# indrajeetadityaroy9/vit-inductive-bias-distillation

Hardware: AMD Instinct MI355X
Metric: distillation images/sec (BASD loss fwd+bwd+grad all-reduce), DeiT-S<-ResNet-50 @ bs256/GPU (higher is better)
Workload: dtype f32; 1 GPU; cfg2 DeiT-S<-ResNet-50 224x224; per_gpu_batch=256, global_batch=256, input_dtype=float32, layout=strided (CLS-sliced / channel-major views), backward=True, grad_allreduce_bytes=88202672, grad_allreduce=none at world size 1 (bucket packed, nothing to exchange), rank_readback=auto, readback_deferred_steps=1756, selector=basd_selector_chain mode 0, parallelism=dp1

## Files before the change

### include/basd_hip.h

```cpp
#ifndef BASD_HIP_H
#define BASD_HIP_H

#include <stdint.h>

#ifdef __cplusplus
extern "C" {
#endif

#ifndef __HIP_PLATFORM_AMD__
typedef struct ihipStream_t* hipStream_t;
#endif

#define BASD_OK 0
#define BASD_EINVAL (-1)
#define BASD_EUNSUPPORTED (-2)
#define BASD_DTYPE_F32 0
#define BASD_DTYPE_BF16 1
#define BASD_DTYPE_U8 2


int basd_gemm_nt(const void* a, int a_dtype, long a_sb, long a_sn, long a_sd, int a_rows_per_batch,
                 long a_batch_stride, const float* b, long ldb, long b_batch_stride, int M, int N, int K, int batch,
                 float* c, long ldc, long c_batch_stride, float scale, const float* bias, float beta,
                 float* colsum_part, float* col_mean, hipStream_t stream);
// ... 80 lines not shown

int basd_grassmann_distance_padded(const float* colnorm, int stride, int n_valid, const int* k_arr, const float* sw,
                                   int sw_stride, const int* sw_index, int items, float* d_out, hipStream_t stream);

int basd_sqrt_clamp(const float* in, float* out, long count, hipStream_t stream);

int basd_gram_finish(const float* c, const float* zbar, int n, int batch, long m_rows, float* out_u, float* out_c,
                     hipStream_t stream);

int basd_selector_tail(const float* t_d, const float* t_e, const float* t_tau, const float* t_vh, const float* t_vals,
                       const float* s_d, const float* s_e, const float* s_tau, const float* s_vh, const float* s_vals,
                       int d_s, int E, int L, int kmax, const int* ranks, const float* proj_s_t, float* z_s,
                       float* v_s, float* z_t, float* u_t, float* u_rot, float* sw, float* cos, int* k_arr,
                       const int* sw_index, float* sigma, int* flags, float* d_out, hipStream_t stream);

int basd_tridiag_mp_rank_rank1(const float* d, const float* e, const float* w, int n, int batch, double rho,
                               double factor, int cap, int* rank_out, const int* status, int* host_mirror,
                               hipStream_t stream);

int basd_tridiag_ranked_gated(float* a, long a_batch_stride, int n, int batch, float* d, float* e, float* tau, float* vh,
                              void* work, int rank_count, double factor, int cap, int* rank_out, int* host_mirror,
                              const unsigned* go_flag, unsigned go_value, int go_budget, hipStream_t stream);
int basd_flag_set(unsigned* flag, unsigned value, hipStream_t stream);

typedef struct BasdSelectorChain {
    const void* const* teacher_host_ptrs;
    long t_dtype, t_sb, t_sn, t_sd;
    const void* const* student_ptrs;
    long s_dtype, s_sb, s_sn, s_sd, s_vec_ok;
    const float* proj_t;
    const float* proj_s_t;
    long E, L, B, n_s, n_t, d_s, d_t;
    double mp_factor;
    long rank_cap;
    long kmax, kmax_cap, mode;
    float* z; float* z_sums; const void* const* z_ptrs; float* z_means; float* t_slabs; long t_splits;
    float* s_partial; float* s_means; float* s_slabs; long s_splits, s_parts;
    float* grams; float* d; float* e; float* tau; float* vh; float* vals; void* tri_work; void* tri_work_s;
    int* ranks; int* host_mirror;
    int* student_status_mirror;
    float* zv; float* vecs; float* u_rot; float* sw; float* cos; float* sigma; float* d_out;
    int* k_arr; const int* sw_index; int* jflags;
    hipStream_t main_stream, chain_stream, student_stream, tail_stream;
    void* ev_fork; void* ev_student; void* ev_ranks; void* ev_tail; void* ev_slot_free; void* ev_tgram; void* ev_tg0;
    hipStream_t fact_stream; unsigned* go_flag; long go_value; long go_budget;
    void* tm_proj; void* tm_tgram; void* tm_scol0; void* tm_scol1; void* tm_sgram; void* tm_tri0; void* tm_mid; void* tm_spec;
    hipStream_t cert_stream; int* cert_mirror; void* ev_cert;
    double* cert_scratch;
} BasdSelectorChain;
int basd_selector_chain(const BasdSelectorChain* args);
int basd_rank_certificate(const float* grams, const float* zbar, int n, int batch, double factor, double* scratch,
                          int* flag, hipStream_t stream);
long basd_rank_certificate_scratch_bytes(int batch);
int basd_debug_fill_lds(unsigned pattern, hipStream_t stream);
int basd_selector_chain_tail(const BasdSelectorChain* args, int kmax, int exact_k);
int basd_jacobi_lds_square_fits(int n);


int basd_token_weights(const void* const* attn_ptrs, int dtype, const float* mix, int L, long sb, long sh, long sq,
                       long sk, int B, int H, int A, int has_cls, int n_a, int n_t, int n_s, const int* atap0,
                       const int* atap1, const float* alam, const int* tap0, const int* tap1, const float* lam,
                       float* omega, float* omega_t, float* raw_out, hipStream_t stream);

int basd_student_project(const void* x, int dtype, long sb, long sn, int B, int n_s, int n_t, int D,
                         const float* omega, const int* tap0, const int* tap1, const float* lam, const int* range0,
                         const int* range1, float* mu, float* tr_s, float* a_prime, hipStream_t stream);

int basd_teacher_center(const void* const* tok_ptrs, int dtype, const float* mix, int L, long sb, long sn, long sd,
                        int B, int n, int D, const int* g0, const int* g1, const float* glam, const float* omega_t,
                        float* mu, float* tc, hipStream_t stream);
int basd_teacher_center_multi(const void* const* tok_ptrs, int dtype, const float* mix, int L, int G, long sb, long sn,
                              long sd, int B, int n, int D, const int* g0, const int* g1, const float* glam,
                              const float* omega_t, float* mu, float* tc, hipStream_t stream);
long basd_teacher_center_stream_scratch_floats(int G, int B, int n, int D);
int basd_teacher_center_stream(const void* const* tok_ptrs, int dtype, const float* mix, int L, int G, long sb, long sn,
                               long sd, int B, int n, int D, const int* g0, const int* g1, const float* glam,
                               const float* omega_t, float* mu, float* tc, float* scratch, hipStream_t stream);

int basd_gram_f64(const float* p, long p_batch_stride, int n, int D, int batch, double* g, long g_batch_stride,
                  hipStream_t stream);

int basd_gram_f64_split(const float* p, long p_batch_stride, int n, int D, int batch, int splits, double* slabs,
                        double* g, hipStream_t stream);

int basd_chol_f64(const double* g, long g_batch_stride, int n, int batch, double* l, long l_batch_stride,
                  hipStream_t stream);

int basd_stack_product(const double* la, const double* lb, long l_batch_stride, int n, int batch, int lb_period,
                       float* w, long w_batch_stride, hipStream_t stream);

int basd_procrustes_finalize(const float* w, long w_batch_stride, const float* sigma, int n, int n_s, int batch,
                             int t_period ,
                             const double* gb, long g_batch_stride, const float* omega, const int* tap0,
                             const int* tap1, const float* lam, const float* tr_s_part, int tr_slabs, float* tr_s,
                             float* tr_t, float* nuc, float* loss, float* k_prime, hipStream_t stream);

int basd_student_project_multi(const void* const* x_ptrs, int dtype, long sb, long sn, int E, int B, int n_s, int n_t,
                               int D, int ptrs_16B_aligned, const float* omega, long omega_e_stride, const int* tap0,
                               const int* tap1, const float* lam, const int* range0, const int* range1, float* mu,
                               float* tr_s, float* a_prime, hipStream_t stream);
int basd_student_grad_multi(const void* const* x_ptrs, int dtype, long sb, long sn, int E, int B, int n_s, int n_t,
                            int D, const float* omega, long omega_e_stride, const float* mu, const float* h,
                            const int* tap0, const int* tap1, const float* lam, const float* scale_ptr,
                            float scale_const, float* dx, const float* tnorm2, float* gomega, hipStream_t stream);
int basd_student_grad_fused(const void* const* x_ptrs, int dtype, long sb, long sn, int E, int B, int n_s, int n_t,
                            int D, int ptrs_16B_aligned, const float* omega, long omega_e_stride, const float* mu,
                            const float* k_prime, const float* a_prime, const int* tap0, const int* tap1,
                            const float* lam, const float* scale_ptr, float scale_const, float* dx,
                            hipStream_t stream);

typedef struct BasdProcrustesArgs {
    const void* const* student_ptrs;
    const void* const* student_host_ptrs;
    long s_dtype, s_sb, s_sn, s_aligned;
    const void* const* tok_ptrs;
    long t_dtype, t_sb, t_sn, t_sd;
    const void* const* attn_ptrs;
    long a_dtype, a_sb, a_sh, a_sq, a_sk;
    const float* mix;
    long E, L, G, B, n_s, n_t, d_s, d_t, H, A, has_cls, n_a, n, max_sweeps;
    const int* atap0; const int* atap1; const float* alam;
    const int* tap0; const int* tap1; const float* lam; const int* range0; const int* range1;
    const int* g0; const int* g1; const float* glam;
    float* omega; float* omega_t; float* raw; float* mu_t; float* tc; float* mu_s; float* tr_part; float* tr_s;
    float* a_prime;
    double* g_all; double* l_all;
    float* W; float* sigma; int* jflags; int* sweeps;
    float* tr_t; float* nuc; float* loss_b; float* k_prime;
    float* h; float* dx; const float* grad_layers;
    double* g_slabs; long g_splits;
    const float* uw_ce; float* uw_out;
    void* jac_ws;
    float* w_stack; float* sigma_u;
} BasdProcrustesArgs;
int basd_procrustes_forward_fused(const BasdProcrustesArgs* args, hipStream_t stream);
int basd_procrustes_tuning(int transposed_cores);

int basd_stack_product_t(const double* la, const double* lb, long l_batch_stride, int n, int batch, int lb_period,
                         float* w, long w_batch_stride, hipStream_t stream);
int basd_kprime_from_transposed(const float* w, long w_batch_stride, const float* sigma, int n, int batch,
                                const double* lb, long l_batch_stride, int lb_period, float* z, long z_batch_stride,
                                float* k_prime, hipStream_t stream);
int basd_procrustes_finish_transposed(const float* w, long w_batch_stride, const float* sigma, int n, int n_s,
                                      int batch, int t_period ,
                                      const double* gb, long g_batch_stride, const float* omega, const int* tap0,
                                      const int* tap1, const float* lam, const float* tr_s_part, int tr_slabs,
                                      float* tr_s, float* tr_t, float* nuc, float* loss, const double* lb,
                                      long l_batch_stride, int lb_period, float* k_prime, hipStream_t stream);
int basd_procrustes_finish_tuning(int fused);
int basd_ustack_stash(const float* wc, long wc_batch_stride, int n, int batch, float* w_stack, long w_stack_stride,
                      hipStream_t stream);
int basd_ustack_from_transposed(const float* x, long x_batch_stride, const float* sigma, int n, int batch,
                                float* w_stack, long w_stack_stride, float* scratch, long scratch_batch_stride,
                                float* sigma_u, int max_sweeps, int* jflags, hipStream_t stream);

int basd_scale_unless_one(float* x, long count, const float* num, const float* den, hipStream_t stream);

int basd_cross_entropy(const void* logits, int dtype, long ld, int B, int C, const long* labels, const float* probs,
                       long pld, float label_smoothing, long ignore_index, float* row_loss, float* dlogits,
                       hipStream_t stream);


int basd_event_create(void** out);
int basd_event_destroy(void* event);
int basd_stream_wait_event(hipStream_t stream, void* event);
int basd_event_record(void* event, hipStream_t stream);
// ... 134 lines not shown
```

### vit-inductive-bias-distillation_amd/basd_amd/_lib.py

```python
from __future__ import annotations

import ctypes as C
import os
import threading

_HERE = os.path.dirname(os.path.abspath(__file__))
LIB_PATH = os.path.join(_HERE, "libbasd_hip.so")

vp, i32, i64, f32, f64 = C.c_void_p, C.c_int, C.c_long, C.c_float, C.c_double

SIGNATURES = {
    "basd_gemm_nt": [vp, i32, i64, i64, i64, i32, i64, vp, i64, i64, i32, i32, i32, i32, vp, i64, i64, f32, vp, f32,
                     vp, vp, vp],
    "basd_gemm_tn_splits": [i32],
    "basd_gemm_tn": [vp, vp, i32, i64, i64, i64, i64, i64, i64, i64, i64, i32, i32, i32, i32, i32, vp, vp, i32, vp,
                     vp, i64, i64, f32, vp],
    "basd_colmean_parts": [i32],
    "basd_colmean": [vp, i32, i64, i64, i64, i32, i64, i32, i32, i32, i32, vp, vp, vp],
    "basd_colmean_multi": [vp, i32, i64, i64, i64, i32, i32, i32, i32, i32, vp, vp, i32, vp],
    "basd_syrk_splits": [i32, i32, i32],
    "basd_syrk_multi": [vp, i32, i64, i64, i64, i32, i32, i32, i32, vp, vp, i32, vp, vp, i64, i32, vp, i32, i32, vp],
    "basd_jacobi_workspace_ints": [i32, i32],
    "basd_jacobi_twopass_workspace_bytes": [i32, i32, i32],
    "basd_jacobi_stacked_twopass": [vp, i64, i32, i32, vp, i32, i32, f32, vp, vp, vp],
    "basd_jacobi_tuning": [i32],
    "basd_jacobi_ordering": [i32],
    "basd_gemm_tuning": [i32],
    "basd_gemm_tuning_get": [],
    "basd_jacobi_onesided": [vp, i64, i32, i32, i32, i32, vp, vp, i32, i32, f32, vp, vp, vp],
    "basd_sort_extract": [vp, i64, i32, i32, i32, i32, vp, i32, vp, vp, i32, vp],
    "basd_tridiag_workspace_bytes": [i32, i32],
    "basd_tridiag_tuning": [i32, i32, i32, i32, i32, i32],
    "basd_tridiag": [vp, i64, i32, i32, vp, vp, vp, vp, vp, vp],
    "basd_tridiag_ranked": [vp, i64, i32, i32, vp, vp, vp, vp, vp, i32, f64, i32, vp, vp, vp, vp],
    "basd_tridiag_ranked_gated": [vp, i64, i32, i32, vp, vp, vp, vp, vp, i32, f64, i32, vp, vp, vp, C.c_uint, i32, vp],
    "basd_flag_set": [vp, C.c_uint, vp],
    "basd_scale_unless_one": [vp, i64, vp, vp, vp],
    "basd_event_create": [vp],
    "basd_event_destroy": [vp],
    "basd_stream_wait_event": [vp, vp],
    "basd_tridiag_eigenvalues": [vp, vp, i32, i32, vp, vp],
    "basd_tridiag_apply_q": [vp, vp, i32, i32, i32, vp, vp, i32, i32, vp],
    "basd_tridiag_shifted_solve": [vp, vp, vp, i32, i32, i32, i32, vp, vp, vp],
    "basd_tridiag_mp_rank": [vp, vp, i32, i32, f64, i32, vp, vp, vp, vp, vp],
    "basd_tridiag_mp_rank_rank1": [vp, vp, vp, i32, i32, f64, f64, i32, vp, vp, vp, vp],
    "basd_tridiag_eigenvectors": [vp, vp, vp, vp, vp, i32, i32, i32, vp, vp, i32, vp],
    "basd_mp_rank": [vp, i32, i32, f64, i32, vp, vp, vp],
    "basd_grassmann_distance": [vp, i32, vp, vp, i32, vp, i32, vp, vp, vp],
    "basd_grassmann_distance_padded": [vp, i32, i32, vp, vp, i32, vp, i32, vp, vp],
    "basd_selector_tail": [vp] * 10 + [i32, i32, i32, i32] + [vp] * 14 + [vp],
    "basd_sqrt_clamp": [vp, vp, i64, vp],
    "basd_gram_finish": [vp, vp, i32, i32, i64, vp, vp, vp],
    "basd_cross_entropy": [vp, i32, i64, i32, i32, vp, vp, i64, f32, i64, vp, vp, vp],
    "basd_token_weights": [vp, i32, vp, i32, i64, i64, i64, i64, i32, i32, i32, i32, i32, i32, i32, vp, vp, vp, vp,
                           vp, vp, vp, vp, vp, vp],
    "basd_student_project": [vp, i32, i64, i64, i32, i32, i32, i32, vp, vp, vp, vp, vp, vp, vp, vp, vp, vp],
    "basd_teacher_center": [vp, i32, vp, i32, i64, i64, i64, i32, i32, i32, vp, vp, vp, vp, vp, vp, vp],
    "basd_teacher_center_multi": [vp, i32, vp, i32, i32, i64, i64, i64, i32, i32, i32, vp, vp, vp, vp, vp, vp, vp],
    "basd_teacher_center_stream_scratch_floats": [i32, i32, i32, i32],
    "basd_teacher_center_stream": [vp, i32, vp, i32, i32, i64, i64, i64, i32, i32, i32, vp, vp, vp, vp, vp, vp, vp, vp],
    "basd_gram_f64": [vp, i64, i32, i32, i32, vp, i64, vp],
    "basd_gram_f64_split": [vp, i64, i32, i32, i32, i32, vp, vp, vp],
    "basd_chol_f64": [vp, i64, i32, i32, vp, i64, vp],
    "basd_stack_product": [vp, vp, i64, i32, i32, i32, vp, i64, vp],
    "basd_procrustes_finalize": [vp, i64, vp, i32, i32, i32, i32, vp, i64, vp, vp, vp, vp, vp, i32, vp, vp, vp, vp,
                                 vp, vp],
    "basd_student_project_multi": [vp, i32, i64, i64, i32, i32, i32, i32, i32, i32, vp, i64, vp, vp, vp, vp, vp, vp,
                                   vp, vp, vp],
    "basd_student_grad_multi": [vp, i32, i64, i64, i32, i32, i32, i32, i32, vp, i64, vp, vp, vp, vp, vp, vp, f32, vp,
                                vp, vp, vp],
    "basd_student_grad_fused": [vp, i32, i64, i64, i32, i32, i32, i32, i32, i32, vp, i64, vp, vp, vp, vp, vp, vp, vp,
                                f32, vp, vp],
    "basd_procrustes_forward_fused": [vp, vp],
    "basd_procrustes_tuning": [i32],
    "basd_jacobi_plain4_fits": [i32],
    "basd_stack_product_t": [vp, vp, i64, i32, i32, i32, vp, i64, vp],
    "basd_kprime_from_transposed": [vp, i64, vp, i32, i32, vp, i64, i32, vp, i64, vp, vp],
    "basd_procrustes_finish_transposed": [vp, i64, vp, i32, i32, i32, i32, vp, i64, vp, vp, vp, vp, vp, i32, vp, vp, vp,
                                          vp, vp, i64, i32, vp, vp],
    "basd_procrustes_finish_tuning": [i32],
    "basd_ustack_stash": [vp, i64, i32, i32, vp, i64, vp],
    "basd_ustack_from_transposed": [vp, i64, vp, i32, i32, vp, i64, vp, i64, vp, i32, vp, vp],
    "basd_resample_tokens": [vp, i32, i64, i64, i64, i32, i32, i32, i32, vp, vp, vp, vp, vp],
    "basd_resample_tokens_adjoint": [vp, i32, i32, i32, i32, vp, vp, vp, vp, vp, vp, vp],
    "basd_teacher_factor": [vp, i64, vp, i32, i32, i32, vp, vp, i64, vp, vp, vp, vp, vp, vp, vp, vp, vp],
    "basd_teacher_factor_tiled": [vp, i64, vp, i32, i32, i32, vp, vp, i64, vp, vp, vp, vp, vp, vp, vp, vp, vp, vp],
    "basd_mix_grad_tokens": [vp, vp, i32, i32, i64, i64, i64, i32, i32, i32, i32, vp, vp, vp, vp, vp],
    "basd_mix_grad_tokens_scratch_floats": [i32, i32, i32, i32],
    "basd_mix_grad_tokens_onepass": [vp, vp, i32, i32, i64, i64, i64, i32, i32, i32, i32, vp, vp, vp, vp, vp, vp],
    "basd_token_weight_bwd": [vp, vp, i32, i32, i32, i32, vp, vp, vp, vp, vp, vp, i32, i32, i64, i64, i64, i64, i32,
                              i32, i32, vp, vp, vp],
    "basd_build_angle_stack": [vp, i32, vp, i32, vp, vp],
    "basd_grassmann_distance_bwd": [vp, vp, i32, vp, vp, i32, vp, vp, i32, vp, vp],
    "basd_eigvec_k2": [vp, vp, i32, i32, i32, vp, vp],
    "basd_selector_chain": [vp],
    "basd_rank_certificate": [vp, vp, i32, i32, f64, vp, vp, vp],
    "basd_rank_certificate_scratch_bytes": [i32],
    "basd_debug_fill_lds": [C.c_uint, vp],
    "basd_selector_chain_tail": [vp, i32, i32],
    "basd_jacobi_lds_square_fits": [i32],
    "basd_event_record": [vp, vp],
    "basd_event_synchronize": [vp],
    "basd_stream_create_priority": [vp, i32],
    "basd_event_create_timed": [vp],
    "basd_event_elapsed_ms": [vp, vp, vp],
    "basd_sfadamw_chunk": [],
    "basd_sfadamw_step": [vp, vp, i32, vp, i32, f32, i32, vp],
    "basd_sfadamw_swap": [vp, vp, i32, vp, i32, vp],
    "basd_sfadamw_launches": [],
    "basd_eval_batch": [vp, i32, i64, i32, i32, vp, i32, vp, f32, i32, vp, vp],
    "basd_mix_batch": [vp, i32, vp, i32, i32, i32, i32, i32, i32, f64, i32, i32, i32, i32, vp, vp, vp, i32, f64, vp,
                       vp],
    "basd_attn_importance": [vp, i32, i64, i64, i32, i32, i32, i32, i32, f32, vp, vp],
    "basd_channel_stats": [vp, i32, i64, i32, i64, vp, i32, vp],
    "basd_trivial_augment": [vp, vp, i32, i32, i32, i32, vp, vp, vp],
}

class ProcrustesArgs(C.Structure):
    _PTRS = ("student_ptrs", "student_host_ptrs")
    _fields_ = (
        [("student_ptrs", vp), ("student_host_ptrs", vp)]
        + [(n, i64) for n in ("s_dtype", "s_sb", "s_sn", "s_aligned")]
        + [("tok_ptrs", vp)] + [(n, i64) for n in ("t_dtype", "t_sb", "t_sn", "t_sd")]
        + [("attn_ptrs", vp)] + [(n, i64) for n in ("a_dtype", "a_sb", "a_sh", "a_sq", "a_sk")]
        + [("mix", vp)]
        + [(n, i64) for n in ("E", "L", "G", "B", "n_s", "n_t", "d_s", "d_t", "H", "A", "has_cls", "n_a", "n",
                              "max_sweeps")]
        + [(n, vp) for n in ("atap0", "atap1", "alam", "tap0", "tap1", "lam", "range0", "range1", "g0", "g1", "glam",
                             "omega", "omega_t", "raw", "mu_t", "tc", "mu_s", "tr_part", "tr_s", "a_prime", "g_all",
                             "l_all", "W", "sigma", "jflags", "sweeps", "tr_t", "nuc", "loss_b", "k_prime", "h", "dx",
                             "grad_layers", "g_slabs")]
        + [("g_splits", i64)]
        + [("uw_ce", vp), ("uw_out", vp), ("jac_ws", vp), ("w_stack", vp), ("sigma_u", vp)]
    )


class SelectorChainArgs(C.Structure):
    _fields_ = (
        [("teacher_host_ptrs", vp)] + [(n, i64) for n in ("t_dtype", "t_sb", "t_sn", "t_sd")]
        + [("student_ptrs", vp)] + [(n, i64) for n in ("s_dtype", "s_sb", "s_sn", "s_sd", "s_vec_ok")]
        + [("proj_t", vp), ("proj_s_t", vp)]
        + [(n, i64) for n in ("E", "L", "B", "n_s", "n_t", "d_s", "d_t")]
        + [("mp_factor", f64)]
        + [(n, i64) for n in ("rank_cap", "kmax", "kmax_cap", "mode")]
        + [(n, vp) for n in ("z", "z_sums", "z_ptrs", "z_means", "t_slabs")] + [("t_splits", i64)]
# ... 63 lines not shown
```

### vit-inductive-bias-distillation_amd/csrc/procrustes.hip

```cpp
#include "basd_common.h"
#include "../../include/basd_hip.h"

namespace basd {

typedef double f64x4 __attribute__((ext_vector_type(4)));

template <typename T>
__global__ void __launch_bounds__(256) token_weights_kernel(const void* const* __restrict__ attn_ptrs,
                                                            const float* __restrict__ mix, int L, long sb, long sh,
                                                            long sq, long sk, int H, int A, int has_cls, int n_a,
                                                            int n_t, int n_s, const int* __restrict__ atap0,
                                                            const int* __restrict__ atap1,
                                                            const float* __restrict__ alam,
                                                            const int* __restrict__ tap0,
                                                            const int* __restrict__ tap1,
                                                            const float* __restrict__ lam, float* __restrict__ omega,
                                                            float* __restrict__ omega_t, float* __restrict__ raw_out) {
    extern __shared__ float sm[];
    float* raw = sm;
    float* w = sm + n_a;
    __shared__ float red[32];
    const int b = blockIdx.x, tid = threadIdx.x;
    for (int j = tid; j < n_a; j += blockDim.x) {
        float acc = 0.f;
// ... 454 lines not shown
    float* out = Tc + gb * n * D + d;
    for (int j = j_lo; j < j_hi; ++j) out[(long)j * D] -= mu;
}

constexpr int G64_BK = 32, G64_LD = 36, G64_TPW = 8;

__global__ void __launch_bounds__(1024) gram_f64_kernel(const float* __restrict__ P, long p_batch_stride, int n, int D,
                                                        double* __restrict__ G, long g_batch_stride,
                                                        long g_split_stride) {
    extern __shared__ __attribute__((aligned(16))) float tile[];
    const int b = blockIdx.x, tid = threadIdx.x, lane = tid & 63, wave = tid >> 6, nw = blockDim.x >> 6;
    G += (long)blockIdx.y * g_split_stride;
    const int nt = (n + 15) / 16, ntiles = nt * (nt + 1) / 2;
    const float* Pb = P + (long)b * p_batch_stride;
    f64x4 acc[G64_TPW];
#pragma unroll
    for (int t = 0; t < G64_TPW; ++t) acc[t] = f64x4{0., 0., 0., 0.};
    int ti[G64_TPW], tj[G64_TPW];
#pragma unroll
    for (int t = 0; t < G64_TPW; ++t) {
        const int lin = wave + (t + (int)blockIdx.z * G64_TPW) * nw;
        int r = 0;
        if (lin < ntiles) {
            r = (int)((sqrtf(8.f * lin + 1.f) - 1.f) * 0.5f);
            while ((r + 1) * (r + 2) / 2 <= lin) ++r;
            while (r * (r + 1) / 2 > lin) --r;
            ti[t] = r;
            tj[t] = lin - r * (r + 1) / 2;
        } else {
            ti[t] = -1;
            tj[t] = -1;
        }
    }
    const int rows_pad = nt * 16;
    const int i16 = lane & 15, kq = lane >> 4;
    for (int k0 = blockIdx.y * G64_BK; k0 < D; k0 += G64_BK * gridDim.y) {
        __syncthreads();
        for (int idx = tid; idx < rows_pad * (G64_BK / 4); idx += blockDim.x) {
            const int r = idx / (G64_BK / 4), c4 = (idx - r * (G64_BK / 4)) * 4, k = k0 + c4;
            float4 v = make_float4(0.f, 0.f, 0.f, 0.f);
            if (r < n) {
                const float* p = Pb + (long)r * D + k;
                if (k + 3 < D) {
                    v = *(const float4*)p;
                } else {
                    if (k < D) v.x = p[0];
                    if (k + 1 < D) v.y = p[1];
                    if (k + 2 < D) v.z = p[2];
                }
            }
            *(float4*)(tile + r * G64_LD + c4) = v;
        }
        __syncthreads();
#pragma unroll
        for (int g = 0; g < G64_BK / 16; ++g) {
#pragma unroll
            for (int t = 0; t < G64_TPW; ++t) {
                if (ti[t] < 0) continue;
                const float4 a = *(const float4*)(tile + (ti[t] * 16 + i16) * G64_LD + g * 16 + 4 * kq);
                const float4 bb = *(const float4*)(tile + (tj[t] * 16 + i16) * G64_LD + g * 16 + 4 * kq);
                acc[t] = __builtin_amdgcn_mfma_f64_16x16x4f64((double)a.x, (double)bb.x, acc[t], 0, 0, 0);
                acc[t] = __builtin_amdgcn_mfma_f64_16x16x4f64((double)a.y, (double)bb.y, acc[t], 0, 0, 0);
                acc[t] = __builtin_amdgcn_mfma_f64_16x16x4f64((double)a.z, (double)bb.z, acc[t], 0, 0, 0);
                acc[t] = __builtin_amdgcn_mfma_f64_16x16x4f64((double)a.w, (double)bb.w, acc[t], 0, 0, 0);
            }
        }
    }
    double* Gb = G + (long)b * g_batch_stride;
#pragma unroll
    for (int t = 0; t < G64_TPW; ++t) {
        if (ti[t] < 0) continue;
        const int col = tj[t] * 16 + (lane & 15);
#pragma unroll
        for (int r = 0; r < 4; ++r) {
            const int row = ti[t] * 16 + (lane >> 4) + 4 * r;
            if (row < n && col < n) {
                Gb[(long)row * n + col] = acc[t][r];
                Gb[(long)col * n + row] = acc[t][r];
            }
        }
    }
}

__global__ void __launch_bounds__(256) gram_f64_reduce_kernel(const double* __restrict__ slabs, long split_stride,
                                                              int splits, long count, double* __restrict__ G) {
    const long i = (long)blockIdx.x * 256 + threadIdx.x;
    if (i >= count) return;
    double acc = 0.;
    for (int s2 = 0; s2 < splits; ++s2) acc += slabs[(long)s2 * split_stride + i];
    G[i] = acc;
}

static bool gram_f64_shape(int n, int* waves, int* chunks, size_t* lds) {
    const int nt = (n + 15) / 16, ntiles = nt * (nt + 1) / 2;
    int w = (ntiles + G64_TPW - 1) / G64_TPW;
    if (w < 4) w = ntiles < 4 ? ntiles : 4;
    int c = 1;
    if (w > 16) {
        c = (ntiles + 16 * G64_TPW - 1) / (16 * G64_TPW);
        w = 16;
    }
    *waves = w;
    *chunks = c;
    *lds = sizeof(float) * (size_t)nt * 16 * G64_LD;
    if (*lds > 156 * 1024) return false;
    if (*lds > 48 * 1024)
        (void)hipFuncSetAttribute((const void*)gram_f64_kernel, hipFuncAttributeMaxDynamicSharedMemorySize, 156 * 1024);
    return true;
}

__device__ __forceinline__ int pk(int i, int j, int n) { return j * n - (j * (j - 1)) / 2 + (i - j); }

__global__ void __launch_bounds__(1024) chol_f64_kernel(const double* __restrict__ G, long g_batch_stride, int n,
                                                        double* __restrict__ Lout, long l_batch_stride) {
    extern __shared__ __attribute__((aligned(16))) double a[];
    double* col = a + (size_t)n * (n + 1) / 2;
    __shared__ double sh_piv;
    __shared__ double red[32];
    const int m = blockIdx.x, tid = threadIdx.x, nthr = blockDim.x, lane = tid & 63, wave = tid >> 6, nw = nthr >> 6;
    const double* Gm = G + (long)m * g_batch_stride;
    double dmax = 0.;
    for (int j = wave; j < n; j += nw)
        for (int i = j + lane; i < n; i += 64) {
            const double v = Gm[(long)i * n + j];
            a[pk(i, j, n)] = v;
            if (i == j) dmax = fmax(dmax, v);
        }
    for (int s = 32; s > 0; s >>= 1) dmax = fmax(dmax, __shfl_xor(dmax, s, 64));
    if (lane == 0) red[wave] = dmax;
    __syncthreads();
    dmax = 0.;
    for (int i = 0; i < nw; ++i) dmax = fmax(dmax, red[i]);
    const double thr = dmax * (double)n * 1e-15;
    for (int j = 0; j < n; ++j) {
        if (tid == 0) {
            const double d = a[pk(j, j, n)];
            sh_piv = d > thr ? sqrt(d) : 0.;
        }
        __syncthreads();
        const double piv = sh_piv;
        const double inv = piv > 0. ? 1. / piv : 0.;
        for (int i = j + tid; i < n; i += nthr) {
            const double v = (i == j) ? piv : a[pk(i, j, n)] * inv;
            a[pk(i, j, n)] = v;
            col[i] = v;
        }
        __syncthreads();
        if (piv > 0.) {
            for (int k = j + 1 + wave; k < n; k += nw) {
                const double ck = col[k];
                for (int i = k + lane; i < n; i += 64) a[pk(i, k, n)] -= col[i] * ck;
            }
        }
        __syncthreads();
    }
    double* Lm = Lout + (long)m * l_batch_stride;
    for (int idx = tid; idx < n * n; idx += nthr) {
        const int i = idx / n, j = idx - i * n;
        Lm[idx] = i >= j ? a[pk(i, j, n)] : 0.;
    }
}

constexpr int CB_NB = 16, CB_KC = 64, CB_MAXR = 16;
__global__ void __launch_bounds__(1024) chol_f64_blocked_kernel(const double* __restrict__ G, long g_batch_stride, int n,
                                                                double* __restrict__ Lout, long l_batch_stride) {
    extern __shared__ __attribute__((aligned(16))) double sm64[];
// ... 824 lines not shown
                if (g < G) chunk_sum[(((long)chunk * G + g) * B + b) * D + d] = musum[g];
        }
        return;
    }
    for (int d = 4 * tid; d < D; d += 1024) {
        float4 musum[TCM_G];
#pragma unroll
        for (int g = 0; g < TCM_G; ++g) musum[g] = make_float4(0.f, 0.f, 0.f, 0.f);
        for (int j = j_lo; j < j_hi; ++j) {
            const long o0 = b * sb + (long)j * sn + d;
            float4 v[TCM_G];
#pragma unroll
            for (int g = 0; g < TCM_G; ++g) v[g] = make_float4(0.f, 0.f, 0.f, 0.f);
            int l = 0;
            for (; l + 4 <= L; l += 4) {
                float4 x[4];
#pragma unroll
                for (int q = 0; q < 4; ++q) x[q] = ld4f((const BASD_GLOBAL_AS float*)tok_ptrs[l + q] + o0);
#pragma unroll
                for (int q = 0; q < 4; ++q)
#pragma unroll
                    for (int g = 0; g < TCM_G; ++g)
                        if (g < G) {
                            const float m = mix[g * L + l + q];
                            v[g].x = fmaf(m, x[q].x, v[g].x); v[g].y = fmaf(m, x[q].y, v[g].y);
                            v[g].z = fmaf(m, x[q].z, v[g].z); v[g].w = fmaf(m, x[q].w, v[g].w);
                        }
            }
            for (; l < L; ++l) {
                const float4 x = ld4f((const BASD_GLOBAL_AS float*)tok_ptrs[l] + o0);
#pragma unroll
                for (int g = 0; g < TCM_G; ++g)
                    if (g < G) {
                        const float m = mix[g * L + l];
                        v[g].x = fmaf(m, x.x, v[g].x); v[g].y = fmaf(m, x.y, v[g].y);
                        v[g].z = fmaf(m, x.z, v[g].z); v[g].w = fmaf(m, x.w, v[g].w);
                    }
            }
#pragma unroll
            for (int g = 0; g < TCM_G; ++g)
                if (g < G) {
                    *(float4*)(Tc + (((long)g * B + b) * n + j) * D + d) = v[g];
                    const float om = omega_t[((long)g * B + b) * n + j];
                    musum[g].x = fmaf(om, v[g].x, musum[g].x); musum[g].y = fmaf(om, v[g].y, musum[g].y);
                    musum[g].z = fmaf(om, v[g].z, musum[g].z); musum[g].w = fmaf(om, v[g].w, musum[g].w);
                }
        }
#pragma unroll
        for (int g = 0; g < TCM_G; ++g)
            if (g < G) *(float4*)(chunk_sum + (((long)chunk * G + g) * B + b) * D + d) = musum[g];
    }
}

long basd_teacher_center_stream_scratch_floats(int G, int B, int n, int D) {
    if (G <= 0 || B <= 0 || n <= 0 || D <= 0) return 0;
    return (long)((n + TCS_ROWS - 1) / TCS_ROWS) * G * B * D;
}
int basd_teacher_center_stream(const void* const* tok_ptrs, int dtype, const float* mix, int L, int G, long sb, long sn,
                               long sd, int B, int n, int D, const int* g0, const int* g1, const float* glam,
                               const float* omega_t, float* mu, float* tc, float* scratch, hipStream_t stream) {
    BASD_CHECK_ARG(tok_ptrs && mix && omega_t && mu && tc && scratch && L > 0 && G > 0 && B > 0 && n > 0 && D > 0);
    BASD_CHECK_ARG((g0 == nullptr) == (g1 == nullptr) && (g0 == nullptr) == (glam == nullptr));
    if (G > TCM_G || sd != 1 || B > 65535 || (long)G * B > 65535) return BASD_EUNSUPPORTED;
    const int chunks = (n + TCS_ROWS - 1) / TCS_ROWS;
    if (dtype == BASD_DTYPE_F32 && g0 == nullptr && D % 4 == 0 && sb % 4 == 0 && sn % 4 == 0 && (((uintptr_t)tc) & 15) == 0 &&
        (((uintptr_t)scratch) & 15) == 0)
        teacher_mix_stream_v4_kernel<<<dim3(chunks, B), 256, 0, stream>>>(tok_ptrs, mix, L, G, sb, sn, n, D, omega_t, tc, scratch);
    else if (dtype == BASD_DTYPE_F32)
        teacher_mix_stream_kernel<float><<<dim3(chunks, B), 256, 0, stream>>>(tok_ptrs, mix, L, G, sb, sn, sd, n, D, g0, g1, glam, omega_t, tc, scratch);
    else if (dtype == BASD_DTYPE_BF16)
        teacher_mix_stream_kernel<__hip_bfloat16><<<dim3(chunks, B), 256, 0, stream>>>(tok_ptrs, mix, L, G, sb, sn, sd, n, D, g0, g1, glam, omega_t, tc, scratch);
    else
        return BASD_EINVAL;
    teacher_center_apply_kernel<<<dim3((D + 255) / 256, chunks, G * B), 256, 0, stream>>>(scratch, chunks, n, D, mu, tc);
    BASD_RETURN_LAST();
}

int basd_gram_f64(const float* p, long p_batch_stride, int n, int D, int batch, double* g, long g_batch_stride,
                  hipStream_t stream) {
    BASD_CHECK_ARG(p && g && n > 0 && D > 0 && batch > 0);
    BASD_CHECK_ARG(((uintptr_t)p & 15) == 0 && D % 4 == 0 && p_batch_stride % 4 == 0);
    int waves, chunks;
    size_t lds;
    if (!gram_f64_shape(n, &waves, &chunks, &lds)) return BASD_EUNSUPPORTED;
    gram_f64_kernel<<<dim3(batch, 1, chunks), 64 * waves, lds, stream>>>(p, p_batch_stride, n, D, g, g_batch_stride, 0);
    BASD_RETURN_LAST();
}

int basd_gram_f64_split(const float* p, long p_batch_stride, int n, int D, int batch, int splits, double* slabs,
                        double* g, hipStream_t stream) {
    BASD_CHECK_ARG(p && g && slabs && n > 0 && D > 0 && batch > 0 && splits >= 1 && splits <= 64);
    BASD_CHECK_ARG(((uintptr_t)p & 15) == 0 && D % 4 == 0 && p_batch_stride % 4 == 0);
    int waves, chunks;
    size_t lds;
    if (!gram_f64_shape(n, &waves, &chunks, &lds)) return BASD_EUNSUPPORTED;
    const long count = (long)batch * n * n;
    gram_f64_kernel<<<dim3(batch, splits, chunks), 64 * waves, lds, stream>>>(p, p_batch_stride, n, D, slabs, (long)n * n, count);
    gram_f64_reduce_kernel<<<(unsigned)((count + 255) / 256), 256, 0, stream>>>(slabs, count, splits, count, g);
    BASD_RETURN_LAST();
}

int basd_chol_f64(const double* g, long g_batch_stride, int n, int batch, double* l, long l_batch_stride,
                  hipStream_t stream) {
    BASD_CHECK_ARG(g && l && n > 0 && batch > 0);
    const size_t lds = sizeof(double) * ((size_t)n * (n + 1) / 2 + n);
    if (lds > 158 * 1024) {
        if (n > 64 * CB_MAXR) return BASD_EUNSUPPORTED;
        const size_t lds_b = sizeof(double) * ((size_t)n * CB_NB + (size_t)CB_NB * (CB_KC + 1));
        (void)hipFuncSetAttribute((const void*)chol_f64_blocked_kernel, hipFuncAttributeMaxDynamicSharedMemorySize, 156 * 1024);
        chol_f64_blocked_kernel<<<batch, 1024, lds_b, stream>>>(g, g_batch_stride, n, l, l_batch_stride);
        BASD_RETURN_LAST();
    }
    (void)hipFuncSetAttribute((const void*)chol_f64_kernel, hipFuncAttributeMaxDynamicSharedMemorySize, 158 * 1024);
    const int threads = n >= 128 ? 1024 : n >= 64 ? 512 : 256;
    chol_f64_kernel<<<batch, threads, lds, stream>>>(g, g_batch_stride, n, l, l_batch_stride);
    BASD_RETURN_LAST();
}

int basd_stack_product(const double* la, const double* lb, long l_batch_stride, int n, int batch, int lb_period,
                       float* w, long w_batch_stride, hipStream_t stream) {
    BASD_CHECK_ARG(la && lb && w && n > 0 && batch > 0 && lb_period > 0);
    const size_t lds = sizeof(double) * 2 * (size_t)n * n;
    if (lds <= 78 * 1024) {
        (void)hipFuncSetAttribute((const void*)stack_product_kernel, hipFuncAttributeMaxDynamicSharedMemorySize, 78 * 1024);
        stack_product_kernel<<<batch, 256, lds, stream>>>(la, lb, l_batch_stride, n, w, w_batch_stride, lb_period);
    } else {
        BASD_CHECK_ARG(batch <= 65535);
        const int nt = (n + 31) / 32;
        stack_product_global_kernel<<<dim3(nt, nt, batch), 256, 0, stream>>>(la, lb, l_batch_stride, n, w, w_batch_stride, lb_period);
    }
    BASD_RETURN_LAST();
}

int basd_stack_product_t(const double* la, const double* lb, long l_batch_stride, int n, int batch, int lb_period,
                         float* w, long w_batch_stride, hipStream_t stream) {
    BASD_CHECK_ARG(la && lb && w && n > 0 && batch > 0 && lb_period > 0 && batch <= 65535);
    const int nt = (n + 31) / 32;
    stack_product_t_kernel<<<dim3(nt, nt, batch), 256, 0, stream>>>(la, lb, l_batch_stride, n, w, w_batch_stride, lb_period);
    BASD_RETURN_LAST();
}

int basd_kprime_from_transposed(const float* w, long w_batch_stride, const float* sigma, int n, int batch,
                                const double* lb, long l_batch_stride, int lb_period, float* z, long z_batch_stride,
                                float* k_prime, hipStream_t stream) {
    BASD_CHECK_ARG(w && sigma && lb && z && k_prime && n > 0 && batch > 0 && lb_period > 0 && batch <= 65535);
    const int nt = (n + 31) / 32;
    kprime_z_kernel<<<dim3(nt, nt, batch), 256, 0, stream>>>(w, w_batch_stride, sigma, n, lb, l_batch_stride, lb_period, z, z_batch_stride);
    kprime_from_z_kernel<<<dim3(nt, nt, batch), 256, 0, stream>>>(z, z_batch_stride, n, k_prime);
    BASD_RETURN_LAST();
}

int basd_ustack_stash(const float* wc, long wc_batch_stride, int n, int batch, float* w_stack, long w_stack_stride,
                      hipStream_t stream) {
    BASD_CHECK_ARG(wc && w_stack && n > 0 && batch > 0 && batch <= 65535 && w_stack_stride >= 2L * n * n);
    m_stash_kernel<<<dim3((unsigned)(((long)n * n + 255) / 256), batch), 256, 0, stream>>>(wc, wc_batch_stride, n, w_stack, w_stack_stride);
    BASD_RETURN_LAST();
}
int basd_ustack_from_transposed(const float* x, long x_batch_stride, const float* sigma, int n, int batch,
                                float* w_stack, long w_stack_stride, float* scratch, long scratch_batch_stride,
                                float* sigma_u, int max_sweeps, int* jflags, hipStream_t stream) {
    BASD_CHECK_ARG(x && sigma && w_stack && scratch && sigma_u && n > 0 && batch > 0 && batch <= 65535 &&
                   w_stack_stride >= 2L * n * n && scratch_batch_stride >= (long)n * n);
    const int nt = (n + 31) / 32;
    ustack_from_x_kernel<<<dim3(nt, nt, batch), 256, 0, stream>>>(x, x_batch_stride, sigma, n, w_stack, w_stack_stride, scratch, scratch_batch_stride);
    int rc = basd_jacobi_onesided(scratch, scratch_batch_stride, n, n, n, batch, nullptr, sigma_u, n, max_sweeps, 0.f,
                                  jflags, nullptr, stream);
    if (rc != BASD_OK) return rc;
    ustack_place_kernel<<<dim3((unsigned)(((long)n * n + 255) / 256), batch), 256, 0, stream>>>(scratch, scratch_batch_stride, n, w_stack, w_stack_stride);
    BASD_RETURN_LAST();
}

int basd_procrustes_finalize(const float* w, long w_batch_stride, const float* sigma, int n, int n_s, int batch,
                             int t_period, const double* gb, long g_batch_stride, const float* omega, const int* tap0,
                             const int* tap1, const float* lam, const float* tr_s_part, int tr_slabs, float* tr_s,
                             float* tr_t, float* nuc, float* loss, float* k_prime, hipStream_t stream) {
    BASD_CHECK_ARG(w && sigma && gb && omega && tr_s_part && tr_s && tr_t && nuc && loss && n > 0 && batch > 0 && tr_slabs > 0);
    BASD_CHECK_ARG(t_period > 0);
    size_t lds = sizeof(float) * ((size_t)n + (k_prime ? (size_t)n * n : 0));
    const bool tiled = lds > 156 * 1024;
    if (tiled) lds = sizeof(float) * (size_t)n;
// ... 127 lines not shown
```

Before: 169,400 images/s.

## Add remainder-aware f64 Gram kernel using MFMA tiles plus scalar edge rows

Adds a specialized f64 Gram kernel for sizes just above a multiple of 16 (n%16 in 1..4, n<=64). It computes the full 16x16 tiles with f64 MFMA and the few leftover rows with per-thread scalar FMA, using double-buffered LDS prefetch. The aim is to avoid padding the whole problem up to the next 16-tile, which wastes MFMA work. It is enabled by default through a toggle, and it adds code paths whose benefit depends on the token count hitting those sizes.

Result: slower. 166,100 images/s (-1.9%).

```diff
diff --git a/include/basd_hip.h b/include/basd_hip.h
--- a/include/basd_hip.h
+++ b/include/basd_hip.h
@@ -186,6 +186,7 @@
 
 int basd_gram_f64_split(const float* p, long p_batch_stride, int n, int D, int batch, int splits, double* slabs,
                         double* g, hipStream_t stream);
+int basd_gram_f64_tuning(int map);
 
 int basd_chol_f64(const double* g, long g_batch_stride, int n, int batch, double* l, long l_batch_stride,
                   hipStream_t stream);
diff --git a/vit-inductive-bias-distillation_amd/basd_amd/_lib.py b/vit-inductive-bias-distillation_amd/basd_amd/_lib.py
--- a/vit-inductive-bias-distillation_amd/basd_amd/_lib.py
+++ b/vit-inductive-bias-distillation_amd/basd_amd/_lib.py
@@ -61,6 +61,7 @@
     "basd_teacher_center_stream": [vp, i32, vp, i32, i32, i64, i64, i64, i32, i32, i32, vp, vp, vp, vp, vp, vp, vp, vp],
     "basd_gram_f64": [vp, i64, i32, i32, i32, vp, i64, vp],
     "basd_gram_f64_split": [vp, i64, i32, i32, i32, i32, vp, vp, vp],
+    "basd_gram_f64_tuning": [i32],
     "basd_chol_f64": [vp, i64, i32, i32, vp, i64, vp],
     "basd_stack_product": [vp, vp, i64, i32, i32, i32, vp, i64, vp],
     "basd_procrustes_finalize": [vp, i64, vp, i32, i32, i32, i32, vp, i64, vp, vp, vp, vp, vp, i32, vp, vp, vp, vp,
diff --git a/vit-inductive-bias-distillation_amd/csrc/procrustes.hip b/vit-inductive-bias-distillation_amd/csrc/procrustes.hip
--- a/vit-inductive-bias-distillation_amd/csrc/procrustes.hip
+++ b/vit-inductive-bias-distillation_amd/csrc/procrustes.hip
@@ -560,6 +560,160 @@
     }
 }
 
+constexpr int G64R_TPW = 2, G64R_PF = 3, G64R_EPT = 4;
+__global__ void __launch_bounds__(192) gram_f64_rem_kernel(const float* __restrict__ P, long p_batch_stride, int n, int D,
+                                                           double* __restrict__ G, long g_batch_stride,
+                                                           long g_split_stride) {
+    extern __shared__ __attribute__((aligned(16))) float tile[];
+    const int b = blockIdx.x, tid = threadIdx.x, lane = tid & 63, wave = tid >> 6, nthr = blockDim.x, nw = nthr >> 6;
+    G += (long)blockIdx.y * g_split_stride;
+    const int nf = n & ~15, rr = n - nf, nft = nf >> 4, ntiles = nft * (nft + 1) / 2;
+    const float* Pb = P + (long)b * p_batch_stride;
+    f64x4 acc[G64R_TPW];
+    int ti[G64R_TPW], tj[G64R_TPW];
+#pragma unroll
+    for (int t = 0; t < G64R_TPW; ++t) {
+        acc[t] = f64x4{0., 0., 0., 0.};
+        const int lin = wave + t * nw;
+        ti[t] = tj[t] = -1;
+        if (lin < ntiles) {
+            ti[t] = lin >= 3 ? 2 : lin >= 1 ? 1 : 0;
+            tj[t] = lin - ti[t] * (ti[t] + 1) / 2;
+        }
+    }
+    const int nrem = rr * nf + rr * (rr + 1) / 2;
+    int ri[G64R_EPT], rj[G64R_EPT];
+    double racc[G64R_EPT];
+#pragma unroll
+    for (int s = 0; s < G64R_EPT; ++s) {
+        int e = tid + s * nthr;
+        ri[s] = rj[s] = -1;
+        racc[s] = 0.;
+        if (e < nrem) {
+            int q = 0;
+            while (e >= nf + q + 1) {
+                e -= nf + q + 1;
+                ++q;
+            }
+            ri[s] = nf + q;
+            rj[s] = e;
+        }
+    }
+    const int i16 = lane & 15, kq = lane >> 4, nvec = n * (G64_BK / 4);
+    float4 pf[G64R_PF];
+    auto fetch = [&](int k0) {
+#pragma unroll
+        for (int p = 0; p < G64R_PF; ++p) {
+            const int idx = tid + p * nthr;
+            float4 v = make_float4(0.f, 0.f, 0.f, 0.f);
+            if (idx < nvec) {
+                const int r = idx / (G64_BK / 4), k = k0 + (idx - r * (G64_BK / 4)) * 4;
+                const float* src = Pb + (long)r * D + k;
+                if (k + 3 < D) {
+                    v = *(const float4*)src;
+                } else {
+                    if (k < D) v.x = src[0];
+                    if (k + 1 < D) v.y = src[1];
+                    if (k + 2 < D) v.z = src[2];
+                }
+            }
+            pf[p] = v;
+        }
+    };
+    auto stash = [&](float* buf) {
+#pragma unroll
+        for (int p = 0; p < G64R_PF; ++p) {
+            const int idx = tid + p * nthr;
+            if (idx < nvec) {
+                const int r = idx / (G64_BK / 4);
+                *(float4*)(buf + r * G64_LD + (idx - r * (G64_BK / 4)) * 4) = pf[p];
+            }
+        }
+    };
+    const int kstep = G64_BK * gridDim.y;
+    int k0 = blockIdx.y * G64_BK, cur = 0;
+    if (k0 < D) {
+        fetch(k0);
+        stash(tile);
+    }
+    __syncthreads();
+    for (; k0 < D; k0 += kstep) {
+        const bool more = k0 + kstep < D;
+        if (more) fetch(k0 + kstep);
+        const float* buf = tile + cur * n * G64_LD;
+#pragma unroll
+        for (int g = 0; g < G64_BK / 16; ++g) {
+#pragma unroll
+            for (int t = 0; t < G64R_TPW; ++t) {
+                if (ti[t] < 0) continue;
+                const float4 a = *(const float4*)(buf + (ti[t] * 16 + i16) * G64_LD + g * 16 + 4 * kq);
+                const float4 bb = *(const float4*)(buf + (tj[t] * 16 + i16) * G64_LD + g * 16 + 4 * kq);
+                acc[t] = __builtin_amdgcn_mfma_f64_16x16x4f64((double)a.x, (double)bb.x, acc[t], 0, 0, 0);
+                acc[t] = __builtin_amdgcn_mfma_f64_16x16x4f64((double)a.y, (double)bb.y, acc[t], 0, 0, 0);
+                acc[t] = __builtin_amdgcn_mfma_f64_16x16x4f64((double)a.z, (double)bb.z, acc[t], 0, 0, 0);
+                acc[t] = __builtin_amdgcn_mfma_f64_16x16x4f64((double)a.w, (double)bb.w, acc[t], 0, 0, 0);
+            }
+        }
+#pragma unroll
+        for (int s = 0; s < G64R_EPT; ++s) {
+            if (s * nthr >= nrem) break;
+            if (ri[s] < 0) continue;
+            const float* pa = buf + ri[s] * G64_LD;
+            const float* pb = buf + rj[s] * G64_LD;
+            double sum = racc[s];
+#pragma unroll
+            for (int g = 0; g < G64_BK / 16; ++g) {
+                float4 a[4], bb[4];
+#pragma unroll
+                for (int q = 0; q < 4; ++q) {
+                    a[q] = *(const float4*)(pa + g * 16 + 4 * q);
+                    bb[q] = *(const float4*)(pb + g * 16 + 4 * q);
+                }
+#pragma unroll
+                for (int q = 0; q < 4; ++q) sum = fma((double)a[q].x, (double)bb[q].x, sum);
+#pragma unroll
+                for (int q = 0; q < 4; ++q) sum = fma((double)a[q].y, (double)bb[q].y, sum);
+#pragma unroll
+                for (int q = 0; q < 4; ++q) sum = fma((double)a[q].z, (double)bb[q].z, sum);
+#pragma unroll
+                for (int q = 0; q < 4; ++q) sum = fma((double)a[q].w, (double)bb[q].w, sum);
+            }
+            racc[s] = sum;
+        }
+        if (more) stash(tile + (cur ^ 1) * n * G64_LD);
+        __syncthreads();
+        cur ^= 1;
+    }
+    double* Gb = G + (long)b * g_batch_stride;
+#pragma unroll
+    for (int t = 0; t < G64R_TPW; ++t) {
+        if (ti[t] < 0) continue;
+        const int col = tj[t] * 16 + (lane & 15);
+#pragma unroll
+        for (int r = 0; r < 4; ++r) {
+            const int row = ti[t] * 16 + (lane >> 4) + 4 * r;
+            Gb[(long)row * n + col] = acc[t][r];
+            Gb[(long)col * n + row] = acc[t][r];
+        }
+    }
+#pragma unroll
+    for (int s = 0; s < G64R_EPT; ++s) {
+        if (ri[s] < 0) continue;
+        Gb[(long)ri[s] * n + rj[s]] = racc[s];
+        Gb[(long)rj[s] * n + ri[s]] = racc[s];
+    }
+}
+
+static int g_gram_map = 1;
+static bool gram_f64_rem_applies(int n) { return g_gram_map && n > 16 && n <= 64 && (n & 15) >= 1 && (n & 15) <= 4; }
+
+static void gram_f64_rem_launch(const float* p, long p_batch_stride, int n, int D, int batch, int splits, double* g,
+                                long g_batch_stride, long g_split_stride, hipStream_t stream) {
+    const int nft = n >> 4, ntiles = nft * (nft + 1) / 2, waves = (ntiles + G64R_TPW - 1) / G64R_TPW;
+    gram_f64_rem_kernel<<<dim3(batch, splits), 64 * waves, sizeof(float) * 2 * (size_t)n * G64_LD, stream>>>(
+        p, p_batch_stride, n, D, g, g_batch_stride, g_split_stride);
+}
+
 __global__ void __launch_bounds__(256) gram_f64_reduce_kernel(const double* __restrict__ slabs, long split_stride,
                                                               int splits, long count, double* __restrict__ G) {
     const long i = (long)blockIdx.x * 256 + threadIdx.x;
@@ -1550,9 +1704,19 @@
     BASD_CHECK_ARG(((uintptr_t)p & 15) == 0 && D % 4 == 0 && p_batch_stride % 4 == 0);
     int waves, chunks;
     size_t lds;
+    if (gram_f64_rem_applies(n)) {
+        gram_f64_rem_launch(p, p_batch_stride, n, D, batch, 1, g, g_batch_stride, 0, stream);
+        BASD_RETURN_LAST();
+    }
     if (!gram_f64_shape(n, &waves, &chunks, &lds)) return BASD_EUNSUPPORTED;
     gram_f64_kernel<<<dim3(batch, 1, chunks), 64 * waves, lds, stream>>>(p, p_batch_stride, n, D, g, g_batch_stride, 0);
     BASD_RETURN_LAST();
+}
+
+int basd_gram_f64_tuning(int map) {
+    const int prev = g_gram_map;
+    if (map >= 0) g_gram_map = map ? 1 : 0;
+    return prev;
 }
 
 int basd_gram_f64_split(const float* p, long p_batch_stride, int n, int D, int batch, int splits, double* slabs,
@@ -1563,7 +1727,10 @@
     size_t lds;
     if (!gram_f64_shape(n, &waves, &chunks, &lds)) return BASD_EUNSUPPORTED;
     const long count = (long)batch * n * n;
-    gram_f64_kernel<<<dim3(batch, splits, chunks), 64 * waves, lds, stream>>>(p, p_batch_stride, n, D, slabs, (long)n * n, count);
+    if (gram_f64_rem_applies(n))
+        gram_f64_rem_launch(p, p_batch_stride, n, D, batch, splits, slabs, (long)n * n, count, stream);
+    else
+        gram_f64_kernel<<<dim3(batch, splits, chunks), 64 * waves, lds, stream>>>(p, p_batch_stride, n, D, slabs, (long)n * n, count);
     gram_f64_reduce_kernel<<<(unsigned)((count + 255) / 256), 256, 0, stream>>>(slabs, count, splits, count, g);
     BASD_RETURN_LAST();
 }
```
